# BrianPugh/tamp

Hardware: AMD Instinct MI355X
Metric: input MB/s, 4KiB-chunk batch compress window=10 (bit-exact vs C ref) (higher is better)
Workload: dtype u8

## Files before the change

### tamp_amd/csrc/tamp_compress_kernel.hpp

```cpp
#pragma once
#include "tamp_common.hpp"

namespace tamp_amd {

constexpr uint32_t kHashBits = 11;
constexpr uint32_t kHashBuckets = 1u << kHashBits;
constexpr uint32_t kRemBits = 16 - kHashBits;
constexpr uint32_t kRunCap = 128;
#ifndef TAMP_LONG_RUN
#define TAMP_LONG_RUN 8
#endif
#ifndef TAMP_DEFER_MIN
#define TAMP_DEFER_MIN 24
#endif
constexpr int kPrioScan = 0, kPrioShort = 2, kPrioWalk = 3;
constexpr uint32_t kDeferMin = TAMP_DEFER_MIN;
constexpr uint32_t kDeferred = 0x1Fu;
constexpr uint32_t kLongRun = TAMP_LONG_RUN;
#ifdef TAMP_SEVEN
#define TAMP_WG_PER_CU 7
constexpr uint32_t kSlowCap = 256, kHb1024 = kHashBits;
#else
constexpr uint32_t kSlowCap = 128;
constexpr uint32_t kHb1024 = 10;
// ... 790 lines not shown
            c_rle = Walk::uni(st_io[W + kSlotRle]), c_ext = Walk::uni(st_io[W + kSlotExtCount]);
            c_nbits = Walk::uni(st_io[W + kSlotNbits]) & 31u;
            c_extpos = Walk::uni((uint32_t)st_io[W + kSlotExtPos] | ((uint32_t)st_io[W + kSlotExtPos + 1] << 8));
            c_bits = Walk::uni((uint32_t)st_io[W + kSlotBits] | ((uint32_t)st_io[W + kSlotBits + 1] << 8) |
                               ((uint32_t)st_io[W + kSlotBits + 2] << 16) | ((uint32_t)st_io[W + kSlotBits + 3] << 24));
        }
        const uint32_t nlead = FXS ? 1u : a.nlead;
        const uint32_t word0 = (BLOCKM && s != 0) ? 0u : (nlead ? (uint32_t)a.lead << 16 : (c_nbits ? c_bits & (0xFFFFFFFFu << (32 - c_nbits)) : 0u));
        for (uint32_t k = tid; k < L.obuf_words; k += nt) obuf[k] = k == 0 ? __builtin_bswap32(word0) : 0;

        Walk wk;
        wk.ebuf = ebuf, wk.blen = blen, wk.bidx = bidx, wk.toklist = toklist, wk.stok = stok;
        wk.W = W, wk.mask = mask, wk.wbits = wbits, wk.lbits = lbits, wk.minp = minp, wk.ext = ext;
        wk.wp_e = wp0, wk.wr = 0, wk.rd = 0, wk.nvalid = 0;
        wk.rle_count = c_rle, wk.ext_count = c_ext, wk.ext_pos = c_extpos, wk.rd = c_rle + c_ext, wk.partial = partial;
        wk.ext_resolved = false, wk.ntok = 0, wk.ns = 0, wk.lane = lane;
        wk.ctlw = (Walk::CtlWord*)ctl, wk.coop = nt == 256;
#ifdef TAMP_PROF
        wk.dbg = a.dbg;
#endif
        wk.lazy = lazy, wk.lazy_valid = false, wk.lazy_idx = 0, wk.lazy_len = 0, wk.blen2 = blen2, wk.bidx2 = bidx2;
        if (tid_k == 0) ctl[cCutThr] = (FXF && FIX == kFixV1) ? 0u : a.cut_run;
        uint32_t w_p0 = bpos;

        uint32_t carry = BLOCKM ? ((uint32_t)(binfo >> 4) & 31u) : (nlead ? 8u * nlead : c_nbits);
        uint32_t gpos = 0;
        uint32_t e_p0 = bpos, e_pending = c_rle + c_ext, e_wp = wp0;
        bool need_match = true;
        uint32_t cur_blk = a_blk;
#ifdef TAMP_PROF
        unsigned long long pt[16] = {0, 0, 0, 0, 0, 0, 0, 0, 0, 0, 0, 0, 0, 0, 0, 0};
        unsigned long long pc = __builtin_readcyclecounter();
#endif
        for (;;) {
            asm volatile("" : "+v"(tid));
            lane = (int)(tid & (kWave - 1)), wave = tid >> 6, wk.lane = lane;
            const uint32_t left = n - e_p0;
            uint32_t nvalid = left < cur_blk ? left : cur_blk;
            if (ext && !LAZY) {
                const uint32_t k0 = W - e_wp;
                if (k0 >= TAMP_ALIGN_MIN && k0 < nvalid) nvalid = k0;
            }
            const uint32_t nplan = nvalid;
            if (!need_match) nvalid = Walk::uni(ctl[cCut]);
            uint32_t nv = LAZY ? 2 * nvalid : nvalid;
            const uint8_t* const steps = LAZY ? vstep : blen;
            if (need_match) {
                __builtin_amdgcn_s_setprio(kPrioShort);
                const uint32_t room = cur_blk + kRing + kPendMax;
                const uint32_t nload = left < room ? left : room;
                TAMP_REPEAT(0x10000u) {
                    const uint8_t* src = in + e_p0;
                    const uint32_t nfill = align_up(nload + 20, 4);
#ifndef TAMP_LOAD_BYTES
                    {
                        const uint32_t nw = nload >> 2;
                        for (uint32_t k = tid; k < nw; k += nt) {
                            uint32_t v;
                            __builtin_memcpy(&v, src + 4 * k, 4);
                            reinterpret_cast<uint32_t*>(ebuf + W)[k] = v;
                        }
                        for (uint32_t k = (nw << 2) + tid; k < nfill; k += nt) ebuf[W + k] = k < nload ? src[k] : 0;
                    }
#else
                    if ((reinterpret_cast<uintptr_t>(src) & 3) == 0) {
                        const uint32_t nw = nload >> 2;
                        for (uint32_t k = tid; k < nw; k += nt)
                            reinterpret_cast<uint32_t*>(ebuf + W)[k] = reinterpret_cast<const uint32_t*>(src)[k];
                        for (uint32_t k = (nw << 2) + tid; k < nfill; k += nt) ebuf[W + k] = k < nload ? src[k] : 0;
                    } else {
                        for (uint32_t k = tid; k < nfill; k += nt) ebuf[W + k] = k < nload ? src[k] : 0;
                    }
#endif
                }
                for (uint32_t k = tid; k < kBuckets / 2; k += nt) cntw[k] = 0;
                if (tid == 0) ctl[cCut] = 0xFFFFFFFFu;
                __syncthreads();
                TAMP_PROF_MARK(0);
#ifdef TAMP_PROF
                pt[12] += 1, pt[13] += nvalid;
#endif

                bool have_tables = false;
                if constexpr (BLOCKM) {
                    have_tables = a.block_pass == 3 && a.blk_len != nullptr;
                    if (have_tables) {
                        const uint8_t* const gl = a.blk_len + bpos;
                        const uint16_t* const gi = a.blk_idx + bpos;
                        for (uint32_t k = tid * 4; k < nvalid; k += nt * 4) {
                            *reinterpret_cast<uint32_t*>(blen + k) = *reinterpret_cast<const uint32_t*>(gl + k);
                            *reinterpret_cast<uint2*>(bidx + k) = *reinterpret_cast<const uint2*>(gi + k);
                        }
                        __syncthreads();
                        for (uint32_t k = nvalid + tid; k < nvalid + 128 && k < a_blk + 128; k += nt) blen[k] = 0x80;
                        __syncthreads();
                    }
                }
                if (!have_tables) {
#ifdef TAMP_PROF
                uint32_t index_reps = (a.dbg & 0x20000u) ? 2u : 1u;
            index_again:
#endif
                asm volatile("" : "+v"(tid));
                lane = (int)(tid & (kWave - 1)), wave = tid >> 6, wk.lane = lane;
                const uint32_t NE0 = nvalid ? W + nvalid : 0;
                const uint32_t cut_run = (FXF && FIX == kFixV1) ? 0u : Walk::uni(ctl[cCutThr]);
                for (uint32_t c4 = tid * 4; c4 < NE0; c4 += nt * 4) {
                    const uint32_t d0 = *reinterpret_cast<const uint32_t*>(ebuf + c4);
                    const uint32_t d1 = *reinterpret_cast<const uint32_t*>(ebuf + c4 + 4);
                    if (d0 == (d0 & 0xFFu) * 0x01010101u) {
                        if constexpr (RUNS) ctl[cQuad] = 1;
                        if (cut_run && d1 == d0 && c4 >= W + e_pending + 4 && c4 + 4 * cut_run <= NE0) {
                            bool all = true;
                            for (uint32_t k = 2; k < cut_run; k++) all = all && *reinterpret_cast<const uint32_t*>(ebuf + c4 + 4 * k) == d0;
                            if (all) atomicMin((uint32_t*)&ctl[cCut], c4);
                        }
                    }
#pragma unroll
                    for (uint32_t j = 0; j < 4; j++) {
                        if (c4 + j < NE0) {
                            const uint32_t h = mix16<HB>(__builtin_amdgcn_alignbyte(d1, d0, j) & 0xFFFFu) >> kRem;
                            atomicAdd(&cntw[h >> 1], 1u << ((h & 1) * 16));
                            if (c4 >= W) qstart[c4 + j - W] = (uint16_t)h;
                        }
                    }
                }
                __syncthreads();
                {
                    const uint32_t cutc = Walk::uni(ctl[cCut]);
                    if (cutc < NE0) nvalid = cutc - W + 4, nv = LAZY ? 2 * nvalid : nvalid;
                }
                const uint32_t NE = nvalid ? W + nvalid : 0;
                for (uint32_t k = nvalid + tid; k < nvalid + 128 && k < a_blk + 128; k += nt) blen[k] = 0x80;
                uint32_t nruns = 0;
                if constexpr (RUNS) {
                    if (Walk::uni(ctl[cQuad])) {
                        for (uint32_t k = tid; k < (W + a_blk + 96) / 32; k += nt) rbits[k] = 0;
                        if (tid == 0) ctl[cNruns] = 0;
                        if (tid < 8) rxset[tid] = 0;
                        __syncthreads();
                        if (tid == 0) ctl[cQuad] = 0;
                        const uint32_t lim = NE + 16;
                        for (uint32_t c = tid; c < NE; c += nt) {
                            const uint32_t b4 = lds_u32_unaligned(ebuf, c), x = b4 & 0xFFu;
                            if (b4 == x * 0x01010101u && (c == 0 || ebuf[c - 1] != x)) {
                                uint32_t e = c + 4;
                                while ((e & 3u) && e < lim && ebuf[e] == x) e++;
                                if (!(e & 3u)) {
                                    while (e + 8 <= lim) {
                                        const uint32_t* wv = reinterpret_cast<const uint32_t*>(ebuf + e);
                                        const uint32_t v0 = wv[0], v1 = wv[1];
                                        if (v0 != b4 || v1 != b4) break;
                                        e += 8;
                                    }
                                    while (e < lim && ebuf[e] == x) e++;
                                }
                                if (e - c >= kLongRun) {
                                    const uint32_t slot = atomicAdd((uint32_t*)&ctl[cNruns], 1u);
                                    if (slot < kRunCap) {
                                        runs[slot] = c | (e << 16);
                                        runsx[slot] = x | ((lds_u32_unaligned(ebuf, e) & 0xFFFFu) << 8);
                                        atomicOr(&rxset[x >> 5], 1u << (x & 31u));
                                        for (uint32_t k = c + 1; k <= e - 4;) {
                                            const uint32_t hiw = min(e - 4, k | 31u);
                                            const uint32_t m = (0xFFFFFFFFu << (k & 31u)) & (0xFFFFFFFFu >> (31u - (hiw & 31u)));
                                            atomicOr(&rbits[k >> 5], m);
// ... 354 lines not shown
                            uint32_t rq = 16;
#pragma unroll
                            for (int jj = 3; jj >= 0; jj--) {
                                const uint32_t xx = P[jj] ^ rep;
                                if (xx) rq = 4u * (uint32_t)jj + ((uint32_t)__builtin_ctz(xx) >> 3);
                            }
                            if (ext && ebuf[W + q - 1] == x && (min(rq, 7u) >= 7u || rq >= R)) continue;
                            const uint32_t cap_len = R < maxp ? R : maxp;
                            const uint32_t sv = blen[q];
                            if ((sv & 0x1Fu) == kDeferred) continue;
                            uint32_t key = (sv & 0x1Fu) ? (((sv & 0x1Fu) << 16) | (W - (uint32_t)bidx[q])) : 0u;
                            const uint32_t key0 = key;
                            bool hit16 = false;
                            {
                                const uint32_t wz = q + W - 16, sh = wz & 31u;
                                uint32_t rb16 = rbits[wz >> 5] >> sh;
                                if (sh > 16) rb16 |= rbits[(wz >> 5) + 1] << (32u - sh);
                                uint32_t wrapmask = (__builtin_bitreverse32(rb16) >> 15) & 0xFFFCu;
                                while (wrapmask) {
                                    const uint32_t t = (uint32_t)__builtin_ctz(wrapmask);
                                    wrapmask &= wrapmask - 1;
                                    const uint32_t c = q + W - t;
                                    if (ebuf[c] != x) continue;
                                    const uint32_t i = (e_wp + c) & mask;
                                    if (i == mask) continue;
                                    const uint32_t lw = prefix_len_wrapped16(ebuf, c, t, W, P);
                                    hit16 = hit16 || lw >= 16;
                                    const uint32_t len = min(lw, min(cap_len, W - i));
                                    const uint32_t k = (len << 16) | (W - i);
                                    if (len >= 2 && k > key) key = k;
                                }
                            }
                            const uint32_t cz = q + ((0u - e_wp - q) & mask);
                            const uint32_t qhi = q + W - 16;
                            const uint32_t pb2 = lds_u32_unaligned(ebuf, W + q + (rq < 16 ? rq : 0u)) & 0xFFFFu;
#pragma unroll 1
                            for (uint32_t k = 0; k < nruns; k++) {
                                const uint32_t rv = Walk::uni(runs[k]), rx = Walk::uni(runsx[k]);
                                const uint32_t ra = rv & 0xFFFFu, rb = rv >> 16;
                                const uint32_t lo = max(ra + 1, q), hi = min(rb - 4, qhi);
                                if ((rx & 0xFFu) != x || lo > hi) continue;
                                const int32_t cs = (int32_t)rb - (int32_t)rq;
                                const bool cz_in = cz >= lo && cz <= hi;
                                {
                                    const int32_t hiA = min((int32_t)hi, cs - 1);
                                    if ((int32_t)lo <= hiA) {
                                        const uint32_t c = cz_in && (int32_t)cz <= hiA ? cz : lo;
                                        const uint32_t lim_i = W - ((c + e_wp) & mask);
                                        key = max(key, (min(rq, min(cap_len, lim_i)) << 16) | lim_i);
                                    }
                                }
                                if (cs >= (int32_t)lo && cs <= (int32_t)hi) {
                                    const uint32_t x2 = (rx >> 8) ^ pb2;
                                    uint32_t len = rq;
                                    if (rq < 16 && !(x2 & 0xFFu)) len = (x2 >> 8) ? rq + 1 : prefix_len16(ebuf, (uint32_t)cs, P);
                                    const uint32_t lim_i = W - (((uint32_t)cs + e_wp) & mask);
                                    key = max(key, (min(len, min(cap_len, lim_i)) << 16) | lim_i);
                                }
                                {
                                    const int32_t c1 = max((int32_t)lo, cs + 1);
                                    if (c1 <= (int32_t)hi) {
                                        const uint32_t lim_i = W - (((uint32_t)c1 + e_wp) & mask);
                                        key = max(key, (min(rb - (uint32_t)c1, min(cap_len, lim_i)) << 16) | lim_i);
                                        if (cz_in && (int32_t)cz > c1) key = max(key, (min(rb - cz, cap_len) << 16) | W);
                                    }
                                }
                            }
                            if (key != key0 || (hit16 && (sv & 0x40u))) {
                                const uint32_t len = key >> 16;
                                const bool slow = (sv & 0x80u) || (ext && len > minp + 11);
                                blen[q] = (uint8_t)(len | (slow ? 0x80u : 0u));
                                bidx[q] = (uint16_t)(W - (key & 0xFFFFu));
                            }
                        }
                    }
                }
                __syncthreads();
                __builtin_amdgcn_s_setprio(kPrioShort);
                TAMP_FINE(f3);
#ifdef TAMP_PROF
                pt[6] += f0, pt[7] += f1, pt[8] += f2, pt[10] += niter;
#endif
                if constexpr (RUNS && PACKED) {
                    if (ext && (kSlowCap * 8 + a_blk) <= (HB == 9 ? kHashBuckets : kBuckets) * 2) {
                        const uint32_t max_ext = minp + 11 + kExtExtraMax;
#ifdef TAMP_PROF
                        for (uint32_t dry = (a.dbg & 0x4000000u) ? 1u : 0u; dry != 0xFFFFFFFFu; dry--)
#else
                        constexpr uint32_t dry = 0;
#endif
                        for (uint32_t q = e_pending + tid; q < nvalid; q += nt) {
                            const uint32_t sv = blen[q];
                            if (!(sv & 0x80u)) continue;
                            const uint32_t len = sv & 0x1Fu;
                            if (len == kDeferred) continue;
                            const uint32_t leftq = n - (e_p0 + q);
                            if (partial && leftq < kRing) continue;
                            const uint32_t wpq = (e_wp + q) & mask;
                            const uint32_t b4 = lds_u32_unaligned(ebuf, W + q - 1);
                            const uint32_t prev = b4 & 0xFFu, b0 = (b4 >> 8) & 0xFFu, b1 = (b4 >> 16) & 0xFFu;
                            if (prev == b0) {
                                if (b1 != b0 || leftq < 2) continue;
                                const uint32_t rep = b0 * 0x01010101u;
                                const uint32_t x0 = lds_u32_unaligned(ebuf, W + q + 2) ^ rep, x1 = lds_u32_unaligned(ebuf, W + q + 6) ^ rep;
                                const uint32_t r = 2u + (x0 ? (uint32_t)__builtin_ctz(x0) >> 3 : 4u + (x1 ? (uint32_t)__builtin_ctz(x1) >> 3 : 4u));
                                if (r > kRleWindowMax || r >= leftq || wpq + r > W) continue;
                                if (r <= 6 && len > r) {
                                    if (len <= minp + 11 && !dry) blen[q] = (uint8_t)len;
                                    continue;
                                }
                                if (!dry) blen[q] = (uint8_t)(0x20u | 1u), xcnt[q] = (uint8_t)r;
                                continue;
                            }
                            if (!(sv & 0x40u)) continue;
                            const uint32_t idx = bidx[q];
                            const uint32_t off = (idx - wpq) & mask, t0 = W - off;
                            const uint32_t lim = min(min(W - idx, max_ext), min(leftq, t0));
                            uint32_t m = 0;
                            while (m < lim) {
                                const uint32_t x = lds_u32_unaligned(ebuf, q + off + m) ^ lds_u32_unaligned(ebuf, W + q + m);
                                if (x) {
                                    m += (uint32_t)__builtin_ctz(x) >> 3;
                                    break;
                                }
                                m += 4;
                            }
                            const uint32_t cnt = min(m, lim);
                            if (cnt >= t0 || cnt < len || wpq + cnt > W) continue;
                            if (partial && leftq < cnt + kRing) continue;
                            if (!dry) blen[q] = (uint8_t)(0x20u | len), xcnt[q] = (uint8_t)cnt;
                        }
                    }
                    __syncthreads();
                }
                }
                for (uint32_t k = 4 + tid; k < 4 + a_blk / 2 && k < L.obuf_words; k += nt) obuf[k] = 0;
                if constexpr (LAZY) {
                    for (uint32_t v = tid; v < nv + 128 && v < 2 * a_blk + 128; v += nt) {
                        uint32_t out = 0x80u;
                        const uint32_t pp = v >> 1, s1 = v & 1u;
                        if (v < nv && pp + 1 < nvalid && !(s1 && pp == 0)) {
                            const uint32_t sva = blen[pp];
                            const uint32_t len = s1 ? (uint32_t)blen2[pp - 1] : (sva & 0x1Fu);
                            if (!(sva & 0x80u) && !(ext && len > minp + 11)) {
                                const uint32_t leftp = n - (e_p0 + pp);
                                const uint32_t R = leftp < kRing ? leftp : kRing;
                                bool defer = false;
                                if (len >= minp && len <= 8 && R > len + 2) {
                                    const uint32_t nlen = blen2[pp], nidx = bidx2[pp];
                                    const uint32_t wpos = (e_wp + pp) & mask;
                                    defer = nlen > len && (wpos < nidx || wpos >= nidx + nlen);
                                }
                                out = defer ? 3u - s1 : 2u * (len >= minp ? len : 1u) - s1;
                            }
                        }
                        vstep[v] = (uint8_t)out;
                    }
                    __syncthreads();
                }
                TAMP_REPEAT(0x40000u)
                for (uint32_t b = wave * 64; b < nv; b += (nt >> 6) * 64) {
                    const uint32_t sv = steps[b + lane];
                    const bool slowp = (sv & 0x80u) != 0;
                    uint32_t stepv = LAZY ? (sv & 0x7Fu) : (sv >= minp ? (sv & 0x1Fu) : 1u);
                    if constexpr (RUNS && PACKED) {
                        if (sv & 0x20u) stepv = xcnt[b + lane];
                        if (b + lane < nv) xcnt[b + lane] = (uint8_t)stepv;
                    }
                    constexpr uint32_t kCnt = (0xFFu << 10) | (BLOCKM ? 0xFFF80000u : 0u);
                    const uint32_t tgt = (uint32_t)lane + stepv;
                    const bool endp = slowp || tgt >= 64u;
                    uint32_t own = 1u << 10;
                    if constexpr (BLOCKM) {
                        const uint32_t lenv = sv & 0x1Fu;
                        own |= (lenv >= minp ? tok_nbits(lenv - minp) + wbits : lbits + 1u) << 19;
                    }
                    uint32_t st = endp ? ((uint32_t)lane << 2) : ((tgt << 2) | own);
                    const uint32_t endv = slowp ? ((uint32_t)lane << 2) : ((tgt << 2) | own);
#pragma unroll
                    for (int r = 0; r < 6; r++) {
                        const uint32_t o2 = (uint32_t)__builtin_amdgcn_ds_bpermute((int)(st & 0x3FFu), (int)st);
                        st = o2 + (st & kCnt);
                    }
                    {
                        const uint32_t e = (uint32_t)__builtin_amdgcn_ds_bpermute((int)(st & 0x3FFu), (int)endv);
                        st = e + (st & kCnt);
                    }
                    if constexpr (BLOCKM) {
                        if (a.block_pass == 1 && b + lane < nv) toklist[b + lane] = (uint16_t)(st >> 19);
                    }
                    st = ((st & 0x3FFu) >> 2) | (((st >> 10) & 0xFFu) << 8);
                    if (b + lane < nv) {
                        if constexpr (LAZY) {
                            jump16[b + lane] = (uint16_t)(b + (st & 0xFFu));
                            count8[b + lane] = (uint8_t)((st >> 8) & 0xFFu);
                        } else {
                            jc32[b + lane] = (b + (st & 0xFFu)) | (((st >> 8) & 0xFFu) << 16);
                        }
                    }
                }
                __syncthreads();
                TAMP_PROF_MARK(2);
            }
            if constexpr (BLOCKM) {
                if (a.block_pass == 1) {
                    if (tid < 16) {
                        uint32_t pos = tid, bits = 0;
                        bool ok = tid < 15;
                        while (ok && pos < nvalid) {
                            const uint32_t jc = jc32[pos], j = jc & 0xFFFFu;
                            if (j == pos) { ok = false; break; }
                            bits += toklist[pos];
                            pos = j;
                        }
                        a.blk_table[(size_t)s * 16 + tid] = ok ? ((pos - nvalid) | (bits << 4)) : 0xFFFFFFFFu;
                    }
                    if (a.blk_len) {
                        uint8_t* const gl = a.blk_len + bpos;
                        uint16_t* const gi = a.blk_idx + bpos;
                        for (uint32_t k = tid * 4; k < nvalid; k += nt * 4) {
                            *reinterpret_cast<uint32_t*>(gl + k) = *reinterpret_cast<const uint32_t*>(blen + k);
                            *reinterpret_cast<uint2*>(gi + k) = *reinterpret_cast<const uint2*>(bidx + k);
                        }
                    }
                    break;
                }
                if (((uint32_t)binfo & 15u) == 15u) {
                    if (s == a.n_blocks - 1 && tid == 0) a.out_len[0] = 0, a.status[0] = kError;
                    break;
                }
                wk.rd = wk.wr = (uint32_t)binfo & 15u;
            }

            if (wave == 0) {
                __builtin_amdgcn_s_setprio(kPrioWalk);
#ifdef TAMP_PROF
                const Walk wk_save = wk;
                uint32_t walk_reps = (a.dbg & 0x8000000u) ? 2u : 1u, ndef = 0;
                bool walk_second = false;
            walk_again:
#endif
                wk.nvalid = nvalid;
                wk.ntok = 0, wk.ns = 0;
                uint32_t act = 0, excess_tok = 0xFFFFFFFFu;
                uint32_t nqueued = 0;
                uint32_t segv = 0;
#ifdef TAMP_PROF
                unsigned long long dbg_list = 0, dbg_hop = 0, dbg_calls = 0;
#endif
// ... 126 lines not shown
                            wk.append(1, wk.wr + 1 == wk.rd, [&](uint32_t) { return c; });
                        } else {
                            wk.emit_rle(wk.rle_count);
                        }
                        wk.rle_count = 0;
                    } else if (!partial && ext && wk.ext_count) {
                        wk.emit_ext();
                    } else {
                        if (st_io && (seg_flags & kSegSave)) {
                            for (uint32_t i = lane; i < W; i += kWave) st_io[i] = (uint8_t)wk.win_l(i);
                            if (lane == 0) {
                                st_io[W + kSlotWindowPos] = (uint8_t)wk.wp();
                                st_io[W + kSlotWindowPos + 1] = (uint8_t)(wk.wp() >> 8);
                                st_io[W + kSlotRle] = (uint8_t)wk.rle_count, st_io[W + kSlotExtCount] = (uint8_t)wk.ext_count;
                                st_io[W + kSlotExtPos] = (uint8_t)wk.ext_pos, st_io[W + kSlotExtPos + 1] = (uint8_t)(wk.ext_pos >> 8);
                                for (uint32_t k = 0; k < 4; k++) st_io[W + kSlotParsed + k] = (uint8_t)(p >> (8 * k));
                            }
                        }
                        act = kActDone;
                        break;
                    }
                }
                list_queued();
#ifdef TAMP_PROF
                if (--walk_reps) {
                    if constexpr (RUNS) {
                        __builtin_amdgcn_wave_barrier();
                        if (lane == 0)
                            for (uint32_t k = 0; k < ndef && k < kRunCap; k++) blen[runs[k]] = (uint8_t)(0x80u | kDeferred);
                        __builtin_amdgcn_wave_barrier();
                    }
                    ndef = 0;
                    wk = wk_save;
                    walk_second = true;
                    goto walk_again;
                }
                if (a.dbg & 0x2000u) wk.dbg_lag_rle += (uint32_t)dbg_hop, wk.dbg_lag_ext += (uint32_t)dbg_list, wk.dbg_lag_rle_short += (uint32_t)dbg_calls;
#endif
                if (act == kActRebase) {
                    const uint32_t pending = wk.rle_count + wk.ext_count;
                    const uint32_t shift = wk.wr;
                    const bool broke = wk.wr + pending != wk.rd;
                    uint32_t nb2 = broke ? max(cur_blk >> TAMP_BRK_SHIFT, (uint32_t)TAMP_BRK_MIN) : min(cur_blk << 1, a_blk);
                    nb2 = min(nb2, a_blk);
                    if (lane == 0) ctl[cBlk] = nb2;
                    if (nvalid < nplan && !broke && wk.rd >= nvalid && lane == 0)
                        ctl[cCutThr] = min(2u * (uint32_t)ctl[cCutThr], 64u);
                    wk.wp_e = wk.wp();
                    w_p0 += wk.rd - pending;
                    wk.wr = 0;
                    wk.rd = pending;
                    if (lane == 0) {
                        ctl[cShift] = shift;
                        ctl[cP0] = w_p0;
                        ctl[cPending] = pending;
                        ctl[cWp] = wk.wp_e;
                    }
                }
                if (lane == 0) {
                    ctl[cAct] = act;
                    ctl[cNtok] = wk.ntok;
                    ctl[cExcess] = excess_tok;
                    ctl[Walk::kCoopCmd] = Walk::kCmdEnd;
                }
                __builtin_amdgcn_s_setprio(kPrioShort);
            } else if (LOOP && tid == 3 * kWave) {
                if (claim[0] == claim[1] && claim[3] == kNoClaim) claim[3] = atomicAdd(a.work_counter, a.claim);
            }
            if (wk.coop && wave != 0)
                wk.serve(wave);
            else
                __syncthreads();
            TAMP_PROF_MARK(3);

#ifdef TAMP_PROF
            uint32_t emit_reps = (a.dbg & 0x80000u) ? 2u : 1u;
        emit_again:
#endif
            asm volatile("" : "+v"(tid));
            lane = (int)(tid & (kWave - 1)), wave = tid >> 6, wk.lane = lane;
            uint32_t act = Walk::uni(ctl[cAct]);
            const uint32_t ntok = Walk::uni(ctl[cNtok]);
            const uint32_t K = (ntok + nt - 1) >> nt_log2;
            const uint32_t k0 = min(tid * K, ntok), k1 = min(k0 + K, ntok);
            auto token = [&](uint32_t k, uint32_t& v, uint32_t& nb) -> bool {
                const uint32_t e = toklist[k];
                if (e & 0x8000u) {
                    v = stok[2 * (e & 0x7FFFu)];
                    nb = stok[2 * (e & 0x7FFFu) + 1];
                    return true;
                }
                uint32_t pos = e, len, idx;
                if (LAZY) {
                    pos = e >> 1;
                    const bool cached = (e & 1u) != 0;
                    const bool deferred = ((e + vstep[e]) & 1u) != 0;
                    len = deferred ? 0u : (cached ? (uint32_t)blen2[pos - 1] : (blen[pos] & 0x1Fu));
                    idx = cached ? (uint32_t)bidx2[pos - 1] : (uint32_t)bidx[pos];
                } else {
                    len = blen[pos] & 0x1Fu, idx = bidx[pos];
                    if constexpr (RUNS && PACKED) {
                        if (blen[pos] & 0x20u) {
                            const uint32_t cnt = xcnt[pos];
                            if (len == 1) {
                                const uint32_t val = cnt - 2, ci = val >> 4;
                                const uint32_t hn = tok_nbits(ci) - 1 + 4;
                                v = ((uint32_t)codetab[kSymRle] << hn) | ((uint32_t)codetab[ci] << 4) | (val & 15u);
                                nb = tok_nbits(kSymRle) + hn;
                            } else {
                                const uint32_t val = cnt - minp - 12, ci = val >> 3;
                                const uint32_t hn = tok_nbits(ci) - 1 + 3;
                                v = ((((uint32_t)codetab[kSymExt] << hn) | ((uint32_t)codetab[ci] << 3) | (val & 7u)) << wbits) | idx;
                                nb = tok_nbits(kSymExt) + hn + wbits;
                            }
                            return true;
                        }
                    }
                }
                if (len < minp) {
                    const uint32_t c = ebuf[W + pos];
                    v = (1u << lbits) | c;
                    nb = lbits + 1;
                    return (c >> lbits) == 0;
                }
                v = ((uint32_t)codetab[len - minp] << wbits) | idx;
                nb = tok_nbits(len - minp) + wbits;
                return true;
            };
            if (lbits < 8) {
                uint32_t v, nb;
                for (uint32_t k = k0; k < k1; k++)
                    if (!token(k, v, nb)) {
                        atomicMin((uint32_t*)&ctl[cExcess], k);
                        break;
                    }
                __syncthreads();
            }
            const uint32_t limit = min((uint32_t)ctl[cExcess], ntok);
            const bool excess = ctl[cExcess] != 0xFFFFFFFFu;
            uint32_t mybits = 0;
#ifndef TAMP_EMIT_TWICE
            const bool tok_cached = K <= 4;
            uint32_t cv[4] = {0, 0, 0, 0}, cn[4] = {0, 0, 0, 0};
            if (tok_cached) {
#pragma unroll
                for (uint32_t j = 0; j < 4; j++) {
                    const uint32_t k = k0 + j;
                    if (k < k1 && k < limit) token(k, cv[j], cn[j]);
                    mybits += cn[j];
                }
            } else
#endif
            for (uint32_t k = k0; k < k1 && k < limit; k++) {
                uint32_t v, nb;
                token(k, v, nb);
                mybits += nb;
            }
            const uint32_t incl = wave_scan_add(mybits);
            if (lane == kWave - 1) ctl[cWave + wave] = incl;
            __syncthreads();
            uint32_t o = carry + incl - mybits, segbits = 0;
            for (uint32_t w2 = 0; w2 < (nt >> 6); w2++) {
                const uint32_t wt = ctl[cWave + w2];
                if (w2 < wave) o += wt;
                segbits += wt;
            }
            {
                uint32_t wi = o >> 5, ph = o & 31, fill = 0;
                uint64_t acc = 0;
                auto put_bits = [&](uint32_t v, uint32_t nb) {
                    acc = (acc << nb) | v;
                    fill += nb;
                    while (ph + fill >= 32) {
                        const uint32_t take = 32 - ph;
                        uint32_t w = (uint32_t)(acc >> (fill - take));
                        if (take < 32) w &= (1u << take) - 1;
                        if (ph == 0)
                            obuf[wi] = __builtin_bswap32(w);
                        else
                            atomicOr(&obuf[wi], __builtin_bswap32(w));
                        fill -= take;
                        ph = 0;
                        wi++;
                    }
                };
#ifndef TAMP_EMIT_TWICE
                if (tok_cached) {
#pragma unroll
                    for (uint32_t j = 0; j < 4; j++)
                        if (cn[j]) put_bits(cv[j], cn[j]);
                } else
#endif
                for (uint32_t k = k0; k < k1 && k < limit; k++) {
                    uint32_t v, nb;
                    token(k, v, nb);
                    put_bits(v, nb);
                }
                if (fill) {
                    const uint32_t w = ((uint32_t)acc & ((1u << fill) - 1)) << (32 - ph - fill);
                    atomicOr(&obuf[wi], __builtin_bswap32(w));
                }
            }
            __syncthreads();
            uint32_t tot = carry + segbits;
            if (excess) act = kActDone;
            if (act == kActDone && !excess && (seg_flags & kSegFlushToken)) {
                const bool want = (tot & 7) != 0 || a.dict_reset;
                if (want && tid == 0) {
                    const uint32_t wi = tot >> 5, ph = tot & 31, v = 0xABu;
                    if (ph + 9 <= 32) {
                        obuf[wi] |= __builtin_bswap32(v << (32 - ph - 9));
                    } else {
                        const uint32_t hi = 32 - ph;
                        obuf[wi] |= __builtin_bswap32(v >> (9 - hi));
                        obuf[wi + 1] |= __builtin_bswap32((v & ((1u << (9 - hi)) - 1)) << (32 - (9 - hi)));
                    }
                }
                if (want) tot += 9;
                if (st_io && tid == 0) st_io[W + kSlotToken] = want ? 1 : 0;
                __syncthreads();
            }
            uint32_t nbytes;
            if (act == kActDone)
                nbytes = (excess || partial) ? (tot >> 3) : ((tot + 7) >> 3);
            else
                nbytes = (tot >> 5) << 2;
            if (act == kActDone && st_io && (seg_flags & kSegSave) && tid == 0) {
                const uint32_t nb = (partial && !excess) ? (tot & 7u) : 0u;
                st_io[W + kSlotNbits] = (uint8_t)nb;
                st_io[W + kSlotBits] = 0, st_io[W + kSlotBits + 1] = 0, st_io[W + kSlotBits + 2] = 0;
                st_io[W + kSlotBits + 3] = nb ? reinterpret_cast<const uint8_t*>(obuf)[tot >> 3] : 0;
            }
            if constexpr (BLOCKM) {
                const uint8_t* ob = reinterpret_cast<const uint8_t*>(obuf);
                const unsigned long long base = ((binfo >> 4) >> 5) << 2;
                const uint32_t c0 = s == 0 ? 0u : carry >> 3, c1 = (tot + 7) >> 3;
                const uint32_t c1c = base + c1 <= cap ? c1 : (base >= cap ? 0u : (uint32_t)(cap - base));
                if (c1c > c0) {
                    uint8_t* const P = gout + base;
                    const uintptr_t A0 = reinterpret_cast<uintptr_t>(P + c0) & ~(uintptr_t)3, A1 = reinterpret_cast<uintptr_t>(P + c1c - 1) & ~(uintptr_t)3;
                    const uint32_t ndw = (uint32_t)((A1 - A0) >> 2) + 1;
                    for (uint32_t j = tid; j < ndw; j += nt) {
                        typedef __attribute__((address_space(1))) uint32_t GlobalWord;
                        GlobalWord* const dst = (GlobalWord*)(A0 + 4 * (uintptr_t)j);
                        const int32_t i0 = (int32_t)((intptr_t)(A0 + 4 * (uintptr_t)j) - reinterpret_cast<intptr_t>(P));
                        uint32_t v = 0;
                        if (i0 >= (int32_t)c0 && i0 + 4 <= (int32_t)c1c) {
                            v = lds_u32_unaligned(ob, (uint32_t)i0);
                        } else {
                            for (int32_t x = 0; x < 4; x++)
                                if (i0 + x >= (int32_t)c0 && i0 + x < (int32_t)c1c) v |= (uint32_t)ob[i0 + x] << (8 * x);
                        }
                        if (j == 0 || j == ndw - 1) __hip_atomic_fetch_or(dst, v, __ATOMIC_RELAXED, __HIP_MEMORY_SCOPE_AGENT);
                        else *dst = v;
                    }
                }
                if (act == kActDone && tid == 0) {
                    const unsigned long long total_bytes = base + c1;
                    a.out_len[0] = total_bytes < cap ? (uint32_t)total_bytes : cap;
                    a.status[0] = total_bytes > cap ? kOutputFull : kOk;
                }
                break;
            }
            {
                const uint8_t* ob = reinterpret_cast<const uint8_t*>(obuf);
                uint8_t* dst = gout + gpos;
                const uint32_t room2 = gpos < cap ? cap - gpos : 0;
                const uint32_t nw = nbytes < room2 ? nbytes : room2;
                const uint32_t head = min((uint32_t)((4 - (reinterpret_cast<uintptr_t>(dst) & 3)) & 3), nw);
                const uint32_t ndw = (nw - head) >> 2;
                if (tid < head) dst[tid] = ob[tid];
                uint32_t* dst32 = reinterpret_cast<uint32_t*>(dst + head);
                for (uint32_t k = tid; k < ndw; k += nt) dst32[k] = lds_u32_unaligned(ob, head + 4 * k);
                for (uint32_t k = head + 4 * ndw + tid; k < nw; k += nt) dst[k] = ob[k];
            }
#ifdef TAMP_PROF
            if (--emit_reps) {
                __syncthreads();
                goto emit_again;
            }
#endif
            if (act == kActDone) {
                if (tid == 0) {
                    const uint32_t total_bytes = gpos + nbytes;
                    a.out_len[s] = total_bytes < cap ? total_bytes : cap;
                    a.status[s] = total_bytes > cap ? kOutputFull : (excess ? kExcessBits : kOk);
                }
                break;
            }
            __syncthreads();
            {
                const uint32_t nfull = tot >> 5;
                const uint32_t lastw = obuf[nfull];
                const uint32_t used = ((tot + 31) >> 5) + 1;
                __syncthreads();
                for (uint32_t k = tid; k < used && k < L.obuf_words; k += nt) obuf[k] = k == 0 ? lastw : 0;
                gpos += nbytes;
                carry = tot & 31;
            }
            TAMP_PROF_MARK(4);
            need_match = act == kActRebase;
            if (act == kActRebase) {
                const uint32_t shift = Walk::uni(ctl[cShift]);
                e_p0 = Walk::uni(ctl[cP0]);
                e_pending = Walk::uni(ctl[cPending]);
                e_wp = Walk::uni(ctl[cWp]);
                cur_blk = Walk::uni(ctl[cBlk]);
                if (shift) {
                    for (uint32_t base = 0; base < W; base += nt * 4) {
                        const uint32_t k = base + tid * 4;
                        uint32_t v = 0;
                        if (k < W) v = lds_u32_unaligned(ebuf, shift + k);
                        __syncthreads();
                        if (k < W) *reinterpret_cast<uint32_t*>(ebuf + k) = v;
                        __syncthreads();
                    }
                }
            }
            __syncthreads();
        }
#ifdef TAMP_PROF
        if (tid == 0 && a.prof) {
            if (a.dbg & 0x3000u) pt[6] = wk.dbg_lag_rle, pt[7] = wk.dbg_lag_ext, pt[8] = wk.dbg_lag_rle_short;
            for (int i = 0; i < 16; i++) atomicAdd(&a.prof[i], pt[i]);
        }
#endif
        if constexpr (LOOP) {
            if (tid_k == 0) {
                uint32_t nx = claim[0];
                if (nx == claim[1]) {
                    nx = claim[3];
                    if (nx == kNoClaim) nx = atomicAdd(a.work_counter, a.claim);
                    claim[1] = nx + a.claim;
                    claim[3] = kNoClaim;
                }
                claim[0] = nx + 1;
                claim[2] = nx;
            }
        }
        __syncthreads();
        if constexpr (!LOOP) break;
    }
}

template <bool PACKED, bool LAZY, bool RUNS = false, uint32_t WSCAN = 0, uint32_t HB = kHashBits, bool LOOP = false, bool BLOCKM = false>
__global__ void __launch_bounds__(256, LAZY ? TAMP_LAZY_PER_CU : (RUNS ? TAMP_WG_PER_CU : TAMP_LEAN_PER_CU)) tamp_compress_kernel(CompressArgs a_k) {
    compress_streams<PACKED, LAZY, RUNS, WSCAN, HB, LOOP, BLOCKM, kFixNone>(a_k);
}

namespace tamp_compress_fixed {
template <uint32_t FIX>
__global__ void __launch_bounds__(256, TAMP_WG_PER_CU) compress_kernel(CompressArgs a_k) {
    static_assert(FIX == kFixExt || FIX == kFixV1, "the generic builds are tamp_compress_kernel's");
    compress_streams<true, false, true, 1u << kFixWbits, kHb1024, true, false, FIX>(a_k);
}
}

}
```

Baseline: 57470.

## Fuse match-extension settle into step scan and restructure bit emission

Removes the separate settle pass over the block tables and its barrier. The settle check now runs inline, per lane, inside the step-table scan, and its count is passed along directly instead of being stored in xcnt and reloaded. Token emission moves from contiguous per-thread ranges to a wave-strided layout with per-row wave scans, and each token is placed with one or two atomicOr calls instead of a per-thread bit accumulator. The global copy-out is done by a single wave using 16-byte stores and now also clears obuf, which removes two __syncthreads. The cost is more atomics on LDS and a narrower copy-out, and correctness now depends on the remaining barriers ordering these steps.

```diff
diff --git a/tamp_amd/csrc/tamp_compress_kernel.hpp b/tamp_amd/csrc/tamp_compress_kernel.hpp
--- a/tamp_amd/csrc/tamp_compress_kernel.hpp
+++ b/tamp_amd/csrc/tamp_compress_kernel.hpp
@@ -896,6 +896,7 @@
 #endif
 
                 bool have_tables = false;
+                bool settle_on = false;
                 if constexpr (BLOCKM) {
                     have_tables = a.block_pass == 3 && a.blk_len != nullptr;
                     if (have_tables) {
@@ -1416,56 +1417,7 @@
                 pt[6] += f0, pt[7] += f1, pt[8] += f2, pt[10] += niter;
 #endif
                 if constexpr (RUNS && PACKED) {
-                    if (ext && (kSlowCap * 8 + a_blk) <= (HB == 9 ? kHashBuckets : kBuckets) * 2) {
-                        const uint32_t max_ext = minp + 11 + kExtExtraMax;
-#ifdef TAMP_PROF
-                        for (uint32_t dry = (a.dbg & 0x4000000u) ? 1u : 0u; dry != 0xFFFFFFFFu; dry--)
-#else
-                        constexpr uint32_t dry = 0;
-#endif
-                        for (uint32_t q = e_pending + tid; q < nvalid; q += nt) {
-                            const uint32_t sv = blen[q];
-                            if (!(sv & 0x80u)) continue;
-                            const uint32_t len = sv & 0x1Fu;
-                            if (len == kDeferred) continue;
-                            const uint32_t leftq = n - (e_p0 + q);
-                            if (partial && leftq < kRing) continue;
-                            const uint32_t wpq = (e_wp + q) & mask;
-                            const uint32_t b4 = lds_u32_unaligned(ebuf, W + q - 1);
-                            const uint32_t prev = b4 & 0xFFu, b0 = (b4 >> 8) & 0xFFu, b1 = (b4 >> 16) & 0xFFu;
-                            if (prev == b0) {
-                                if (b1 != b0 || leftq < 2) continue;
-                                const uint32_t rep = b0 * 0x01010101u;
-                                const uint32_t x0 = lds_u32_unaligned(ebuf, W + q + 2) ^ rep, x1 = lds_u32_unaligned(ebuf, W + q + 6) ^ rep;
-                                const uint32_t r = 2u + (x0 ? (uint32_t)__builtin_ctz(x0) >> 3 : 4u + (x1 ? (uint32_t)__builtin_ctz(x1) >> 3 : 4u));
-                                if (r > kRleWindowMax || r >= leftq || wpq + r > W) continue;
-                                if (r <= 6 && len > r) {
-                                    if (len <= minp + 11 && !dry) blen[q] = (uint8_t)len;
-                                    continue;
-                                }
-                                if (!dry) blen[q] = (uint8_t)(0x20u | 1u), xcnt[q] = (uint8_t)r;
-                                continue;
-                            }
-                            if (!(sv & 0x40u)) continue;
-                            const uint32_t idx = bidx[q];
-                            const uint32_t off = (idx - wpq) & mask, t0 = W - off;
-                            const uint32_t lim = min(min(W - idx, max_ext), min(leftq, t0));
-                            uint32_t m = 0;
-                            while (m < lim) {
-                                const uint32_t x = lds_u32_unaligned(ebuf, q + off + m) ^ lds_u32_unaligned(ebuf, W + q + m);
-                                if (x) {
-                                    m += (uint32_t)__builtin_ctz(x) >> 3;
-                                    break;
-                                }
-                                m += 4;
-                            }
-                            const uint32_t cnt = min(m, lim);
-                            if (cnt >= t0 || cnt < len || wpq + cnt > W) continue;
-                            if (partial && leftq < cnt + kRing) continue;
-                            if (!dry) blen[q] = (uint8_t)(0x20u | len), xcnt[q] = (uint8_t)cnt;
-                        }
-                    }
-                    __syncthreads();
+                    settle_on = ext && (kSlowCap * 8 + a_blk) <= (HB == 9 ? kHashBuckets : kBuckets) * 2;
                 }
                 }
                 for (uint32_t k = 4 + tid; k < 4 + a_blk / 2 && k < L.obuf_words; k += nt) obuf[k] = 0;
@@ -1492,13 +1444,73 @@
                     }
                     __syncthreads();
                 }
+                auto settle = [&](uint32_t q, uint32_t sv, uint32_t& cnt_out) -> uint32_t {
+                    const uint32_t max_ext = minp + 11 + kExtExtraMax;
+                    const uint32_t len = sv & 0x1Fu;
+                    if (len == kDeferred) return sv;
+                    const uint32_t leftq = n - (e_p0 + q);
+                    if (partial && leftq < kRing) return sv;
+                    const uint32_t wpq = (e_wp + q) & mask;
+                    const uint32_t b4 = lds_u32_unaligned(ebuf, W + q - 1);
+                    const uint32_t prev = b4 & 0xFFu, b0 = (b4 >> 8) & 0xFFu, b1 = (b4 >> 16) & 0xFFu;
+                    if (prev == b0) {
+                        if (b1 != b0 || leftq < 2) return sv;
+                        const uint32_t rep = b0 * 0x01010101u;
+                        const uint32_t x0 = lds_u32_unaligned(ebuf, W + q + 2) ^ rep, x1 = lds_u32_unaligned(ebuf, W + q + 6) ^ rep;
+                        const uint32_t r = 2u + (x0 ? (uint32_t)__builtin_ctz(x0) >> 3 : 4u + (x1 ? (uint32_t)__builtin_ctz(x1) >> 3 : 4u));
+                        if (r > kRleWindowMax || r >= leftq || wpq + r > W) return sv;
+                        if (r <= 6 && len > r)
+                            return len <= minp + 11 ? len : sv;
+                        cnt_out = r;
+                        return 0x20u | 1u;
+                    }
+                    if (!(sv & 0x40u)) return sv;
+                    const uint32_t idx = bidx[q];
+                    const uint32_t off = (idx - wpq) & mask, t0 = W - off;
+                    const uint32_t lim = min(min(W - idx, max_ext), min(leftq, t0));
+                    uint32_t m = 0;
+                    while (m < lim) {
+                        const uint32_t x = lds_u32_unaligned(ebuf, q + off + m) ^ lds_u32_unaligned(ebuf, W + q + m);
+                        if (x) {
+                            m += (uint32_t)__builtin_ctz(x) >> 3;
+                            break;
+                        }
+                        m += 4;
+                    }
+                    const uint32_t cnt = min(m, lim);
+                    if (cnt >= t0 || cnt < len || wpq + cnt > W) return sv;
+                    if (partial && leftq < cnt + kRing) return sv;
+                    cnt_out = cnt;
+                    return 0x20u | len;
+                };
+#ifdef TAMP_PROF
+                if (settle_on && (a.dbg & 0x4000000u))
+                    for (uint32_t q = wave * 64 + lane; q < nvalid; q += nt) {
+                        const uint32_t sv = blen[q];
+                        if (!(sv & 0x80u) || q < e_pending) continue;
+                        uint32_t c = 0;
+                        const uint32_t sv2 = settle(q, sv, c);
+                        asm volatile("" ::"v"(sv2), "v"(c));
+                    }
+#endif
                 TAMP_REPEAT(0x40000u)
                 for (uint32_t b = wave * 64; b < nv; b += (nt >> 6) * 64) {
-                    const uint32_t sv = steps[b + lane];
+                    uint32_t sv = steps[b + lane];
+                    uint32_t settled = 0;
+                    if constexpr (RUNS && PACKED) {
+                        if (settle_on && (sv & 0x80u) && b + lane >= e_pending && b + lane < nvalid) {
+                            const uint32_t sv2 = settle(b + lane, sv, settled);
+                            if (sv2 != sv) blen[b + lane] = (uint8_t)sv2;
+                            sv = sv2;
+                        }
+                    }
                     const bool slowp = (sv & 0x80u) != 0;
                     uint32_t stepv = LAZY ? (sv & 0x7Fu) : (sv >= minp ? (sv & 0x1Fu) : 1u);
                     if constexpr (RUNS && PACKED) {
-                        if (sv & 0x20u) stepv = xcnt[b + lane];
+                        if (sv & 0x20u) stepv = settled;
+#ifdef TAMP_PROF
+                        if ((sv & 0x20u) && !settled) stepv = xcnt[b + lane];
+#endif
                         if (b + lane < nv) xcnt[b + lane] = (uint8_t)stepv;
                     }
                     constexpr uint32_t kCnt = (0xFFu << 10) | (BLOCKM ? 0xFFF80000u : 0u);
@@ -1791,7 +1803,7 @@
             uint32_t act = Walk::uni(ctl[cAct]);
             const uint32_t ntok = Walk::uni(ctl[cNtok]);
             const uint32_t K = (ntok + nt - 1) >> nt_log2;
-            const uint32_t k0 = min(tid * K, ntok), k1 = min(k0 + K, ntok);
+            const uint32_t kb = wave * (K << 6) + (uint32_t)lane;
             auto token = [&](uint32_t k, uint32_t& v, uint32_t& nb) -> bool {
                 const uint32_t e = toklist[k];
                 if (e & 0x8000u) {
@@ -1838,76 +1850,73 @@
             };
             if (lbits < 8) {
                 uint32_t v, nb;
-                for (uint32_t k = k0; k < k1; k++)
-                    if (!token(k, v, nb)) {
+                for (uint32_t j = 0; j < K; j++) {
+                    const uint32_t k = kb + (j << 6);
+                    if (k < ntok && !token(k, v, nb)) {
                         atomicMin((uint32_t*)&ctl[cExcess], k);
                         break;
                     }
+                }
                 __syncthreads();
             }
             const uint32_t limit = min((uint32_t)ctl[cExcess], ntok);
             const bool excess = ctl[cExcess] != 0xFFFFFFFFu;
-            uint32_t mybits = 0;
 #ifndef TAMP_EMIT_TWICE
-            const bool tok_cached = K <= 4;
-            uint32_t cv[4] = {0, 0, 0, 0}, cn[4] = {0, 0, 0, 0};
-            if (tok_cached) {
+            constexpr uint32_t kEmitRows = 2;
+#else
+            constexpr uint32_t kEmitRows = 0;
+#endif
+            uint32_t cv[kEmitRows + 1], cn[kEmitRows + 1];
+            uint32_t run = 0;
 #pragma unroll
-                for (uint32_t j = 0; j < 4; j++) {
-                    const uint32_t k = k0 + j;
-                    if (k < k1 && k < limit) token(k, cv[j], cn[j]);
-                    mybits += cn[j];
-                }
-            } else
-#endif
-            for (uint32_t k = k0; k < k1 && k < limit; k++) {
-                uint32_t v, nb;
-                token(k, v, nb);
-                mybits += nb;
-            }
-            const uint32_t incl = wave_scan_add(mybits);
-            if (lane == kWave - 1) ctl[cWave + wave] = incl;
+            for (uint32_t j = 0; j < kEmitRows; j++) {
+                cv[j] = 0, cn[j] = 0;
+                if (j < K) {
+                    const uint32_t k = kb + (j << 6);
+                    uint32_t v = 0, nb = 0;
+                    if (k < limit) token(k, v, nb);
+                    const uint32_t incl = wave_scan_add(nb);
+                    cv[j] = v, cn[j] = nb | ((run + incl - nb) << 6);
+                    run += (uint32_t)__builtin_amdgcn_readlane((int)incl, kWave - 1);
+                }
+            }
+            const uint32_t runc = run;
+            for (uint32_t j = kEmitRows; j < K; j++) {
+                const uint32_t k = kb + (j << 6);
+                uint32_t v = 0, nb = 0;
+                if (k < limit) token(k, v, nb);
+                run += (uint32_t)__builtin_amdgcn_readlane((int)wave_scan_add(nb), kWave - 1);
+            }
+            if (lane == 0) ctl[cWave + wave] = run;
             __syncthreads();
-            uint32_t o = carry + incl - mybits, segbits = 0;
+            uint32_t o = carry, segbits = 0;
             for (uint32_t w2 = 0; w2 < (nt >> 6); w2++) {
                 const uint32_t wt = ctl[cWave + w2];
                 if (w2 < wave) o += wt;
                 segbits += wt;
             }
             {
-                uint32_t wi = o >> 5, ph = o & 31, fill = 0;
-                uint64_t acc = 0;
-                auto put_bits = [&](uint32_t v, uint32_t nb) {
-                    acc = (acc << nb) | v;
-                    fill += nb;
-                    while (ph + fill >= 32) {
-                        const uint32_t take = 32 - ph;
-                        uint32_t w = (uint32_t)(acc >> (fill - take));
-                        if (take < 32) w &= (1u << take) - 1;
-                        if (ph == 0)
-                            obuf[wi] = __builtin_bswap32(w);
-                        else
-                            atomicOr(&obuf[wi], __builtin_bswap32(w));
-                        fill -= take;
-                        ph = 0;
-                        wi++;
+                auto put_token = [&](uint32_t v, uint32_t nb, uint32_t p) {
+                    if (nb) {
+                        const uint64_t x = (uint64_t)v << (64u - (p & 31u) - nb);
+                        const uint32_t hi = (uint32_t)(x >> 32), lo = (uint32_t)x;
+                        atomicOr(&obuf[p >> 5], __builtin_bswap32(hi));
+                        if (lo) atomicOr(&obuf[(p >> 5) + 1], __builtin_bswap32(lo));
                     }
                 };
-#ifndef TAMP_EMIT_TWICE
-                if (tok_cached) {
 #pragma unroll
-                    for (uint32_t j = 0; j < 4; j++)
-                        if (cn[j]) put_bits(cv[j], cn[j]);
-                } else
-#endif
-                for (uint32_t k = k0; k < k1 && k < limit; k++) {
-                    uint32_t v, nb;
-                    token(k, v, nb);
-                    put_bits(v, nb);
-                }
-                if (fill) {
-                    const uint32_t w = ((uint32_t)acc & ((1u << fill) - 1)) << (32 - ph - fill);
-                    atomicOr(&obuf[wi], __builtin_bswap32(w));
+                for (uint32_t j = 0; j < kEmitRows; j++)
+                    if (j < K) put_token(cv[j], cn[j] & 63u, o + (cn[j] >> 6));
+                if (K > kEmitRows) {
+                    uint32_t run2 = o + runc;
+                    for (uint32_t j = kEmitRows; j < K; j++) {
+                        const uint32_t k = kb + (j << 6);
+                        uint32_t v = 0, nb = 0;
+                        if (k < limit) token(k, v, nb);
+                        const uint32_t incl = wave_scan_add(nb);
+                        put_token(v, nb, run2 + incl - nb);
+                        run2 += (uint32_t)__builtin_amdgcn_readlane((int)incl, kWave - 1);
+                    }
                 }
             }
             __syncthreads();
@@ -1971,17 +1980,34 @@
                 }
                 break;
             }
-            {
+#ifdef TAMP_PROF
+            const bool last_rep = emit_reps == 1;
+#else
+            constexpr bool last_rep = true;
+#endif
+            if (wave == (nt >> 6) - 1) {
                 const uint8_t* ob = reinterpret_cast<const uint8_t*>(obuf);
                 uint8_t* dst = gout + gpos;
                 const uint32_t room2 = gpos < cap ? cap - gpos : 0;
                 const uint32_t nw = nbytes < room2 ? nbytes : room2;
                 const uint32_t head = min((uint32_t)((4 - (reinterpret_cast<uintptr_t>(dst) & 3)) & 3), nw);
-                const uint32_t ndw = (nw - head) >> 2;
-                if (tid < head) dst[tid] = ob[tid];
-                uint32_t* dst32 = reinterpret_cast<uint32_t*>(dst + head);
-                for (uint32_t k = tid; k < ndw; k += nt) dst32[k] = lds_u32_unaligned(ob, head + 4 * k);
-                for (uint32_t k = head + 4 * ndw + tid; k < nw; k += nt) dst[k] = ob[k];
+                const uint32_t nch = (nw - head) >> 4, r0 = head + (nch << 4);
+                const uint32_t ndw = (nw - r0) >> 2, t0 = r0 + (ndw << 2);
+                struct __attribute__((packed, aligned(4))) GlobalU128 { uint32_t x, y, z, w; };
+                if ((uint32_t)lane < head) dst[lane] = ob[lane];
+                for (uint32_t c = (uint32_t)lane; c < nch; c += kWave) {
+                    const LdsU128 v = *reinterpret_cast<const LdsU128*>(ob + head + (c << 4));
+                    *reinterpret_cast<GlobalU128*>(dst + head + (c << 4)) = GlobalU128{v.x, v.y, v.z, v.w};
+                }
+                if ((uint32_t)lane < ndw) *reinterpret_cast<uint32_t*>(dst + r0 + 4 * lane) = lds_u32_unaligned(ob, r0 + 4 * lane);
+                if (t0 + (uint32_t)lane < nw) dst[t0 + lane] = ob[t0 + lane];
+                if (act != kActDone && last_rep) {
+                    asm volatile("" ::: "memory");
+                    const uint32_t lastw = obuf[tot >> 5];
+                    const uint32_t used4 = min((((tot + 31) >> 5) + 1 + 3) >> 2, (L.obuf_words + 3) >> 2);
+                    for (uint32_t c = (uint32_t)lane; c < used4; c += kWave)
+                        reinterpret_cast<uint4*>(obuf)[c] = make_uint4(c == 0 ? lastw : 0u, 0u, 0u, 0u);
+                }
             }
 #ifdef TAMP_PROF
             if (--emit_reps) {
@@ -1997,16 +2023,8 @@
                 }
                 break;
             }
-            __syncthreads();
-            {
-                const uint32_t nfull = tot >> 5;
-                const uint32_t lastw = obuf[nfull];
-                const uint32_t used = ((tot + 31) >> 5) + 1;
-                __syncthreads();
-                for (uint32_t k = tid; k < used && k < L.obuf_words; k += nt) obuf[k] = k == 0 ? lastw : 0;
-                gpos += nbytes;
-                carry = tot & 31;
-            }
+            gpos += nbytes;
+            carry = tot & 31;
             TAMP_PROF_MARK(4);
             need_match = act == kActRebase;
             if (act == kActRebase) {
```

Result: faster. 58100 (median of 6 runs) (+1.1%).
